# marvinx97/cloud

Measured on AMD Instinct MI355X. Metric: images/sec ResNet-50 via run() at 1/2/4/8 MI355X; run()→first-step latency, higher is better.
Workload: dtype bf16

## Files before the change

cloud_amd/config.py:

```python
from __future__ import annotations

import os
from dataclasses import dataclass


@dataclass(frozen=True)
class Var:
    name: str
    type: type
    default: object
    doc: str
    area: str


_VARS = [
    Var("CLOUD_AMD_JOBS_DIR", str, "./jobs", "where run() stages job directories", "launcher"),
    Var("CLOUD_AMD_HOME", str, "~/.cloud_amd", "per-user state: the job-id index (jobs/<id> -> job directory) that "
        "python -m cloud_amd.jobs uses to find a job from any directory", "launcher"),
    Var("CLOUD_AMD_STAGE_COPY", bool, False, "stage code files by copying too (default: code "
        "hard-linked, every other file copied; a running job then never sees in-place edits of its sources)", "launcher"),
    Var("CLOUD_AMD_CPU_AFFINITY", bool, True, "launcher pins each GPU rank to the cores of its GPU's NUMA node "
        "(KFD io_links + sysfs cpulist), split between the ranks on that node; 0 = leave placement to the OS",
        "launcher"),
    Var("CLOUD_AMD_NUMA_ROOT", str, "/sys/devices/system/node", "sysfs NUMA-node tree read for rank CPU placement "
# ... 27 lines not shown
        "core of ca_gemm256p8.h for large GEMMs), 'glds' (128 core only), 'vp8' (the two-phase 256 core whenever "
        "M, N >= 256), 'reg' (register staging); any other name selects 'auto'", "ops"),
    Var("CLOUD_AMD_WGRAD_BLOCKS", int, 512, "convolution weight gradients: split-K so that about this many "
        "workgroups run (tiles x splits); fewer splits = less fp32 slab traffic, more = fuller CUs", "ops"),
    Var("CLOUD_AMD_WGRAD_BLOCKS_SMALLM", int, 512, "convolution weight gradients with <= 128 output channels "
        "(ResNet stem, layers 1-2): split-K workgroup target", "ops"),
    Var("CLOUD_AMD_STEM_WGRAD_BLOCKS", int, 2048, "space-to-depth stem weight gradient (the last kernel of the "
        "backward pass): split-K workgroup target", "ops"),
    Var("CLOUD_AMD_DENSE_WGRAD_BLOCKS", int, 640, "dense-layer weight gradients (BERT): split-K workgroup target "
        "(round 4, same box: 640 -> 6,993 / 6,993 seq/s, 768 -> 6,962 / 6,952, 1024 -> 6,892 / 6,911, 512 -> "
        "6,865 / 6,896; profiles/r4_s36/)",
        "ops"),
    Var("CLOUD_AMD_DENSE_WGRAD_256", bool, False, "dense-layer weight gradients whose 256 x 256 tiles times a split "
        "count fill one round of the chip (BERT QKV / FFN) run on the two-phase 256 core with that split (measured "
        "3 % slower on BERT than the 128 core's 1024-workgroup split: 6,749 / 6,754 vs 6,952 / 6,940 seq/s)", "ops"),
    Var("CLOUD_AMD_TAPMASK", bool, True, "convolutions: tap-mask / incremental buffer-mode gather loaders; 0 keeps "
        "the general per-chunk decode loaders (A/B runs)", "ops"),
    Var("CLOUD_AMD_SPLIT_XCD", bool, True, "split-K GEMM/conv grids: give each XCD contiguous (split, tile) "
        "ranges so the tiles of one K chunk share an L2; 0 remaps tiles only (A/B runs)", "ops"),
    Var("CLOUD_AMD_BN_APPLY_BLOCKS", int, 0, "BatchNorm apply passes (fwd y/mask, bwd dz): total workgroups of "
        "the HBM stream; 0 = the reduction kernels' tiling", "ops"),
    Var("CLOUD_AMD_BN_APPLY_ILV", bool, True, "BatchNorm apply passes: 1 = RP-row groups dealt round-robin to "
        "the workgroups (one contiguous sweep); 0 = one contiguous row chunk per workgroup", "ops"),
    Var("CLOUD_AMD_CONV_TALL", bool, True, "<= 64-channel 3x3 convolutions (fwd, stride-1 dgrad): 256 x 64 tiles "
        "with 4 x 1 waves; 0 = 128 x 64 with 2 x 2 waves", "ops"),
    Var("CLOUD_AMD_STEM_LDS", bool, True, "space-to-depth stem convolution forward on the LDS-resident patch + filter "
        "kernel (csrc/include/ca_conv_stem.h); 0 = the implicit-GEMM row-segment loader", "ops"),
    Var("CLOUD_AMD_STEM_TALL", bool, True, "space-to-depth stem convolution on the tall 256 x 64 tiles too (0.88 -> "
        "0.72 ms per call at b1024); 0 = 128 x 64 tiles (A/B runs)", "ops"),
    Var("CLOUD_AMD_STEM_BWD_RECOMPUTE", bool, True, "ResNet stem tail backward: a statistics-only max-pool "
        "backward pass, then the BN-backward apply recomputes the pooled gradient per 2x2 block (the 112x112 "
        "gradient is never written: 3.3 GB fewer per step at b1024).  With the window loads issued ahead of "
        "any branch: 0.65 + 0.90 ms against 1.09 + 0.94 for write-then-apply, +0.8 % end to end "
        "(profiles/r4_s44/); 0 = write g and run the separate apply pass", "ops"),
    Var("CLOUD_AMD_BN_GROUPS_MAX", int, 512, "BatchNorm statistics: most groups of the first-level reduction of the "
        "per-tile partial rows (1..512; ~64 rows per group)", "ops"),
    Var("CLOUD_AMD_GEMM_LIB", str, "never", "plain bf16 GEMMs (bias / accumulate only, no fused epilogue): 'never' "
        "(default: every GEMM on the in-tree kernels, the same engine on every box and rank), 'auto' (diagnostic: "
        "times the in-tree kernel against hipBLASLt once per shape and keeps the faster), 'always' "
        "(ops/raw.py PlainGemmPolicy)", "ops"),
    Var("CLOUD_AMD_GEMM_PRW", bool, True, "forward 1x1 convolutions with N = 256, K = 64 (ResNet layer-1 conv3 "
        "and shortcut): persistent resident-weight core (csrc/include/ca_gemm_prw.h); 0 = the tiled 128 core",
        "ops"),
    Var("CLOUD_AMD_GEMM_PRWN", bool, True, "forward 1x1 convolutions N = 512 / K = 128 and N = 1024 / K = 256 with "
        "BN statistics (ResNet stage-2 / stage-3 conv3): the persistent core with the weight resident in column "
        "chunks (ca_gemm_prw.h); 0 = the tiled 128 core", "ops"),
    Var("CLOUD_AMD_SMALLK_SET", str, "", "bench/smallk_gemm.py shape set ('conv3': the conv3 expansions of "
        "stages 2-4)", "bench"),
    Var("CLOUD_AMD_EPI_PF", bool, True, "GEMM epilogues that read memory or run an activation (BN-statistics "
        "and inference-BN forward 1x1 convs, BERT bias/GELU/GELU'/beta dense layers): 4 staged output rows in flight per trip", "ops"),
    Var("CLOUD_AMD_EPI_PIPE", bool, True, "input-gradient GEMMs / convolutions with the BN-backward statistics "
        "epilogue: the next two output rows' operand loads are in flight under this pair's arithmetic and stores "
        "(ca_mfma_core.h gemm_epilogue); 0 = one pair at a time (A/B runs)", "ops"),
    Var("CLOUD_AMD_ATTN_FUSED_BWD", bool, True,"attention at S = 64 / 128: one workgroup per (batch, head) for "
        "the forward and a single fused backward kernel; 0 keeps the 64-query-block kernels", "ops"),
    Var("CLOUD_AMD_CONV_HALO_WGRAD", bool, True, "the weight gradient of the same 3x3 / 64-channel / width-56 "
        "convolutions on the LDS-resident kernel (ca_conv_halo.h conv3x3_halo_wgrad: 64 x 576 partial in registers, "
        "one fp32 slab per workgroup); 0 = implicit GEMM (A/B)", "ops"),
    Var("CLOUD_AMD_LN_BWD16", bool, False, "LayerNorm backward on 16-wave blocks, one row per wave, the block's "
        "partials summed by a fixed LDS tree (measured 2.8 % slower on BERT beside the weight-gradient side stream; "
        "default: 4-wave blocks walking four rows per wave)", "ops"),
    Var("CLOUD_AMD_GEMM_256X96", bool, True, "forward GEMMs whose 256 x 96 grid fills whole rounds while the 128 x "
        "128 grid leaves a partial one (BERT QKV, M = 8192, N = 2304) run on 256 x 96 tiles; 0 = off (A/B)", "ops"),
    Var("CLOUD_AMD_BN_FIN_RPG", int, 512, "BatchNorm statistics finalize: partial rows per group block (64-512)", "ops"),
    Var("CLOUD_AMD_BN_FIN_MERGED", bool, True, "BatchNorm statistics from many partial rows: group reduction and "
        "per-channel finalize in ONE launch (last block per 64 channels finalizes, agent-scope ticket); 0 = two "
        "launches (A/B runs)", "ops"),
    Var("CLOUD_AMD_CONV_HALO", int, 1, "3x3 / stride-1 / 64-channel convolutions at width 56 (ResNet-50 "
        "stage 1) forward and input gradient on the LDS-resident kernel (ca_conv_halo.h: input patch and all 9 taps "
        "in LDS, persistent grid); 0 = implicit-GEMM tiles, 2 = halo kernel without the software-pipelined "
        "fragment reads (A/B runs)", "ops"),
    Var("CLOUD_AMD_CONV_PATCH", bool, True, "3x3 / stride-1 / pad-1 convolutions with a 64-multiple gathered channel "
        "count, more than 64 output columns and W <= 28 (ResNet-50 stages 2-4), forward and input gradient, on the "
        "patch-fed core (ca_conv_patch.h: the tile's input rows go to LDS once per 64-channel chunk, not once per "
        "tap); 0 = tap-gathered implicit GEMM (A/B runs)", "ops"),
    Var("CLOUD_AMD_CONV_EPI_PF", bool, True, "implicit-GEMM forward convolutions with the BN-statistics epilogue, and "
        "with the inference BN + residual + ReLU epilogue: read 2 staged output rows from LDS before storing", "ops"),
    Var("CLOUD_AMD_INFER_FUSE", bool, True, "ResNet blocks and stem that are not training (eval mode, or a frozen "
        "Keras base) under torch.no_grad(): every BatchNorm (+ residual + ReLU) in the epilogue of its convolution "
        "(ops.conv_bn_act_infer, ca_conv_fwd_bn) and no BN-statistics partials; 0 = the per-layer route "
        "(convolution with statistics, then bn_apply)", "ops"),
    Var("CLOUD_AMD_SHAPE_LOG", str, None, "profiling: append one JSON line per GEMM/convolution launch (kind, M, N, "
        "K, minimum HBM bytes) to this file, for scripts/gemm_roofline.py", "ops"),
    Var("CLOUD_AMD_BN_FOLD", bool, True, "ResNet block backward: the bn3 / bn1 backward apply runs in the operand "
        "fetch of the 1x1 input-gradient GEMM that consumes it (ca_gemm_xa.h) instead of a separate pass", "ops"),
    Var("CLOUD_AMD_BN_FOLD_FWD", bool, True, "ResNet block forward: bn2's apply runs in conv3's operand fetch and "
        "bn3's (+ residual) in the next block's conv1 (ca_gemm_xa.h); the applied tensors are written once, by "
        "those GEMMs", "ops"),
    Var("CLOUD_AMD_BN_FOLD_MAX_N", int, 256, "BN fold sites kept: only GEMMs with K >= 2N and N <= this "
        "(ResNet-50 default: bn3 -> conv3 dgrad and bn3 -> next conv1 at stages 1-3, the stage-3 ones on the two-deep "
        "128 x 256 transform-A tiles, CLOUD_AMD_XA_N256=3: +0.6 / +1.0 % on two boxes, docs/performance.md round 6; "
        "4096 = every stage); the short-K sites (bn2 -> conv3, bn1 -> conv1 dgrad) measured slower than the separate "
        "pass, and stage 4 (N 512) +0.3 % below stages 1-3 only", "ops"),
    Var("CLOUD_AMD_BN_FOLD_WGRAD", bool, True, "bn3 -> conv3 fold at 64 input channels (ResNet stage 1): conv3's weight "
        "gradient runs in the same kernel as its input gradient (ca_gemm_xa.h mfma_gemm_xa_dw), so the BN-backward "
        "output dz3 is never written", "ops"),
    Var("CLOUD_AMD_BN_FOLD_DS", bool, False, "ResNet projection blocks, stages 2-4: the shortcut BN's backward apply "
        "runs in the operand fetch of the sparse strided shortcut input-gradient GEMM (ca_gemm_xa_bwd_strided); A/B",
        "ops"),
    Var("CLOUD_AMD_DS_SPARSE_DGRAD", bool, True, "ResNet projection blocks with a strided 1x1 shortcut: the "
        "shortcut's input gradient is written for its one non-empty output-parity class only, and conv1's input "
        "gradient accumulates into it reading the other pixels as zeros -- no zero-fill of 3/4 of dx and no read "
        "of those zeros", "ops"),
    Var("CLOUD_AMD_BN_FOLD_WGRAD_DS", bool, True, "stage-1 projection shortcut: its BN backward (gated by the block "
        "output's ReLU mask), the shortcut conv's input gradient and its weight gradient in one pass", "ops"),
    Var("CLOUD_AMD_BN_FOLD_WGRAD2", bool, False, "the same one-pass input + weight gradient for stage 2's conv3 "
# ... 166 lines not shown
```

csrc/bindings.cpp:

```cpp
#include <atomic>
#include <mutex>
#include <hip/hip_runtime.h>
#include <pybind11/pybind11.h>
#include <pybind11/stl.h>
#include <stdint.h>

#include <stdexcept>
#include <string>
#include <vector>

namespace py = pybind11;
typedef uint16_t bf16_t;

extern "C" {
int ca_sgd_step(float*, void*, int, float*, bf16_t*, const float*, const float*, long, int, int, hipStream_t);
int ca_adam_step(float*, void*, int, float*, float*, bf16_t*, const float*, const float*, long, int, int, hipStream_t);
int ca_rmsprop_step(float*, void*, int, float*, float*, bf16_t*, const float*, const float*, long, int, hipStream_t);
int ca_sumsq(const void*, int, long, float*, hipStream_t);
int ca_scale(void*, int, long, const float*, hipStream_t);
long ca_bn_workspace_floats(long, int);
int ca_bn_fwd(const bf16_t*, const bf16_t*, bf16_t*, long, int, const float*, const float*, float, float,
              float*, float*, float*, float*, float*, float*, int, uint8_t*, hipStream_t);
int ca_bn_apply(const bf16_t*, const bf16_t*, bf16_t*, long, int, const float*, int, hipStream_t);
int ca_bn_fwd_partials(const bf16_t*, const bf16_t*, bf16_t*, long, int, const float*, int, const float*, const float*,
// ... 21 lines not shown
                           hipStream_t);
int ca_gemm_xa_dw(const bf16_t*, const bf16_t*, const uint8_t*, const float*, const float*, const float*, long,
                  const bf16_t*, long, bf16_t*, long, int, int, int, float, const bf16_t*, const uint8_t*,
                  const bf16_t*, const uint8_t*, float*, const bf16_t*, float*, const bf16_t*, long, void*, int, float,
                  float*, int, hipStream_t);
int ca_dgrad_gemm(int, const bf16_t*, long, const bf16_t*, long, bf16_t*, long, int, int, int, float, const bf16_t*,
                  const uint8_t*, const bf16_t*, const uint8_t*, float*, hipStream_t, const bf16_t*, float*, int, int,
                  int);
int ca_conv_dgrad_bnstats(const bf16_t*, const bf16_t*, bf16_t*, int, int, int, int, int, int, int, int, int, int,
                          int, float, const bf16_t*, const uint8_t*, float*, hipStream_t);
int ca_u8_normalize(const uint8_t*, bf16_t*, long, int, const float*, const float*, hipStream_t);
int ca_stem_s2d(const bf16_t*, bf16_t*, int, int, int, int, int, int, int, hipStream_t);
int ca_softmax_xent(const void*, int, const int64_t*, int, int, float, float, float*, float*, void*, hipStream_t);
int ca_softmax_xent_batch(const void*, long, int, const int64_t*, int, int, float, float, float*, float*, void*, float*,
                          float,
                          hipStream_t);
int ca_maxpool_fwd(const bf16_t*, bf16_t*, uint8_t*, int, int, int, int, int, int, int, int, int, hipStream_t);
int ca_maxpool_bwd(const bf16_t*, const uint8_t*, bf16_t*, int, int, int, int, int, int, int, int, int, hipStream_t);
int ca_gap_fwd(const bf16_t*, void*, int, int, int, int, hipStream_t);
int ca_gap_bwd(const void*, int, bf16_t*, int, int, int, hipStream_t);
int ca_gmp_fwd(const bf16_t*, bf16_t*, float*, int, int, int, hipStream_t);
int ca_gmp_bwd(const void*, int, const bf16_t*, const bf16_t*, const float*, bf16_t*, int, int, int, hipStream_t);
int ca_gemm_bf16(int, const bf16_t*, long, const bf16_t*, long, bf16_t*, long, int, int, int, float*, float,
                 hipStream_t);
int ca_gemm_set_core(int);
int ca_gemm_set_xa_n256(int);
int ca_gemm_stat_rows(int, int, int, long, long, long);
int ca_bn_relu_maxpool_s2k3(const bf16_t*, const float*, bf16_t*, uint8_t*, int, int, int, int, int, int, hipStream_t);
int ca_maxpool_bnstats_parts(int, int, int, int);
int ca_maxpool_bwd_s2k3_bnstats(const bf16_t*, const bf16_t*, const uint8_t*, const bf16_t*, bf16_t*, float*, int, int,
                                int, int, int, int, hipStream_t);
int ca_maxpool_bwd_s2k3_bnapply(const bf16_t*, const bf16_t*, const uint8_t*, const bf16_t*, const float*, bf16_t*, int,
                                int, int, int, int, int, hipStream_t);
int ca_conv_fwd_ex(const bf16_t*, const bf16_t*, bf16_t*, int, int, int, int, int, int, int, int, int, int, int,
                   const float*, int, hipStream_t);
int ca_conv_fwd(const bf16_t*, const bf16_t*, bf16_t*, int, int, int, int, int, int, int, int, int, int, int, float*,
                hipStream_t);
int ca_conv_fwd_bn(const bf16_t*, const bf16_t*, bf16_t*, int, int, int, int, int, int, int, int, int, int, int,
                   const float*, const float*, const bf16_t*, int, hipStream_t);
int ca_conv_dgrad(const bf16_t*, const bf16_t*, bf16_t*, int, int, int, int, int, int, int, int, int, int, int, float,
                  hipStream_t, int);
int ca_conv_wgrad(const bf16_t*, const bf16_t*, void*, int, float, int, int, int, int, int, int, int, int, int, int,
                  int, int, float*, hipStream_t);
int ca_splitk_reduce(const float*, int, long, void*, int, float, hipStream_t);
int ca_grad_finalize_multi(const uint64_t*, const float*, int, hipStream_t);
int ca_cls_head_max_labels();
int ca_cls_head_fwd(const bf16_t*, long, const float*, const float*, float*, int, int, int, float, uint64_t,
                    hipStream_t);
int ca_cls_head_bwd(const float*, const bf16_t*, long, const float*, bf16_t*, float*, float*, int, int, int, float,
                    uint64_t, hipStream_t);
int ca_gemm_splitk(int, const bf16_t*, long, const bf16_t*, long, void*, int, float, int, int, int, int, float*,
                   hipStream_t);
int ca_gemm_splitk_effective(int, int);
int ca_gemm_ex(int, const bf16_t*, long, const bf16_t*, long, bf16_t*, long, int, int, int, float*, float, const float*,
               int, bf16_t*, const bf16_t*, long, hipStream_t);
long ca_ln_workspace_floats(long, int);
int ca_ln_fwd(const bf16_t*, const bf16_t*, const float*, const float*, bf16_t*, bf16_t*, float*, float*, long, int,
              float, float, uint64_t, float, uint64_t, const float*, hipStream_t);
int ca_ln_bwd(const bf16_t*, const bf16_t*, const float*, const float*, const float*, bf16_t*, bf16_t*, float*, float*,
              int, float*, long, int, float, uint64_t, float, uint64_t, hipStream_t, float*);
long ca_colsum_workspace_floats(long, int);
int ca_colsum(const bf16_t*, long, int, long, float*, int, float*, hipStream_t);
int ca_act_grad(const bf16_t*, long, int, const bf16_t*, bf16_t*, long, int, int, hipStream_t);
int ca_pad_cols(const void*, long, int, void*, int, long, long, int, hipStream_t);
int ca_slice_acc(const float*, long, void*, int, long, int, hipStream_t);
int ca_pad_cols_multi(const long*, int, hipStream_t);
int ca_splitk_bias_act(const float*, int, long, int, const float*, int, bf16_t*, hipStream_t);
int ca_embed_sum(const int32_t*, const int32_t*, const float*, const float*, const float*, bf16_t*, long, int, int, int,
                 hipStream_t);
int ca_embed_bwd(const bf16_t*, const int32_t*, const int32_t*, float*, float*, float*, long, int, int, int, int, int,
                 int, float*, unsigned*, hipStream_t);
int ca_dropout(const bf16_t*, bf16_t*, long, float, uint64_t, hipStream_t);
int ca_dropout_mask(uint8_t*, long, long, float, uint64_t, hipStream_t);
int ca_attn_fwd(const bf16_t*, bf16_t*, float*, const int*, int, int, int, float, float, uint64_t, int, hipStream_t);
int ca_attn_bwd(const bf16_t*, const bf16_t*, const bf16_t*, const float*, float*, bf16_t*, const int*, int, int, int,
                float, float, uint64_t, int, hipStream_t);
}

#define P(T, x) reinterpret_cast<T>(static_cast<uintptr_t>(x))
#define S(x) reinterpret_cast<hipStream_t>(static_cast<uintptr_t>(x))

static void check(int rc, const char* what) {
  if (rc != 0) {
    std::string msg = std::string(what) + " failed: ";
    if (rc > 0) msg += hipGetErrorString(static_cast<hipError_t>(rc));
    else if (rc == -3)
      msg += "an operand window of one GEMM block exceeds the 2 GiB reach of the buffer loads (split the batch or K)";
    else msg += "invalid arguments (code " + std::to_string(rc) + ")";
    throw std::runtime_error(msg);
  }
}

typedef unsigned long long u64;

static int stream_wait(u64 dst, u64 src) {
  static hipEvent_t ring[16];
  static std::atomic<int> next{0};
  static std::once_flag once;
  static hipError_t init_err = hipSuccess;
  std::call_once(once, [] {
    for (auto& e : ring) {
      const hipError_t rc = hipEventCreateWithFlags(&e, hipEventDisableTiming);
      if (rc != hipSuccess) init_err = rc;
    }
  });
  if (init_err != hipSuccess) return (int)init_err;
// ... 214 lines not shown
  });
  m.def("maxpool_bwd_s2k3_bnapply", [](u64 dy, u64 yp, u64 idx, u64 z, u64 coef, u64 dz, int N, int H, int W, int C,
                                       int OH, int OW, u64 s) {
    check(ca_maxpool_bwd_s2k3_bnapply(P(const bf16_t*, dy), P(const bf16_t*, yp), P(const uint8_t*, idx),
                                      P(const bf16_t*, z), P(const float*, coef), P(bf16_t*, dz), N, H, W, C, OH, OW,
                                      S(s)),
          "maxpool_bwd_s2k3_bnapply");
  });
  m.def("conv_fwd_ex", [](u64 x, u64 w, u64 y, int Nb, int H, int W, int Cin, int Cout, int KH, int KW, int sh,
                          int sw, int ph, int pw, u64 bias, int act, u64 s) {
    check(ca_conv_fwd_ex(P(const bf16_t*, x), P(const bf16_t*, w), P(bf16_t*, y), Nb, H, W, Cin, Cout, KH, KW, sh, sw,
                         ph, pw, P(const float*, bias), act, S(s)), "conv_fwd_ex");
  });
  m.def("conv_dgrad", [](u64 dy, u64 w, u64 dx, int Nb, int H, int W, int Cin, int Cout, int KH, int KW, int sh,
                         int sw, int ph, int pw, float beta, u64 s, int skip_empty) {
    check(ca_conv_dgrad(P(const bf16_t*, dy), P(const bf16_t*, w), P(bf16_t*, dx), Nb, H, W, Cin, Cout, KH, KW, sh, sw,
                        ph, pw, beta, S(s), skip_empty), "conv_dgrad");
  }, py::arg("dy"), py::arg("w"), py::arg("dx"), py::arg("Nb"), py::arg("H"), py::arg("W"), py::arg("Cin"),
        py::arg("Cout"), py::arg("KH"), py::arg("KW"), py::arg("sh"), py::arg("sw"), py::arg("ph"), py::arg("pw"),
        py::arg("beta"), py::arg("s"), py::arg("skip_empty") = 0);
  m.def("conv_wgrad", [](u64 dy, u64 x, u64 dw, int dw_bf16, float beta, int Nb, int H, int W, int Cin, int Cout,
                         int KH, int KW, int sh, int sw, int ph, int pw, int splits, u64 ws, u64 s) {
    check(ca_conv_wgrad(P(const bf16_t*, dy), P(const bf16_t*, x), P(void*, dw), dw_bf16, beta, Nb, H, W, Cin, Cout,
                        KH, KW, sh, sw, ph, pw, splits, P(float*, ws), S(s)), "conv_wgrad");
  });
  m.def("grad_finalize_multi", [](const std::vector<uint64_t>& jobs, const std::vector<float>& betas, u64 s) {
    const int n = (int)betas.size();
    if ((long)jobs.size() != 12L * n) throw std::runtime_error("grad_finalize_multi: 12 fields per job");
    check(ca_grad_finalize_multi(jobs.data(), betas.data(), n, S(s)), "grad_finalize_multi");
  });
  m.def("cls_head_max_labels", []() { return ca_cls_head_max_labels(); });
  m.def("cls_head_fwd", [](u64 pooled, long ldp, u64 wc, u64 bc, u64 logits, int B, int C, int L, float p, u64 seed,
                           u64 s) {
    check(ca_cls_head_fwd(P(const bf16_t*, pooled), ldp, P(const float*, wc), P(const float*, bc), P(float*, logits),
                          B, C, L, p, seed, S(s)), "cls_head_fwd");
  });
  m.def("cls_head_bwd", [](u64 dl, u64 pooled, long ldp, u64 wc, u64 dpre, u64 gwc, u64 gbc, int B, int C, int L,
                           float p, u64 seed, u64 s) {
    check(ca_cls_head_bwd(P(const float*, dl), P(const bf16_t*, pooled), ldp, P(const float*, wc), P(bf16_t*, dpre),
                          P(float*, gwc), P(float*, gbc), B, C, L, p, seed, S(s)), "cls_head_bwd");
  });
  m.def("splitk_reduce", [](u64 ws, int splits, long MN, u64 out, int out_bf16, float beta, u64 s) {
    check(ca_splitk_reduce(P(const float*, ws), splits, MN, P(void*, out), out_bf16, beta, S(s)), "splitk_reduce");
  });
  m.def("gemm_splitk", [](int layout, u64 A, long lda, u64 B, long ldb, u64 out, int out_bf16, float beta, int M,
                          int N, int K, int splits, u64 ws, u64 s) {
    check(ca_gemm_splitk(layout, P(const bf16_t*, A), lda, P(const bf16_t*, B), ldb, P(void*, out), out_bf16, beta,
                         M, N, K, splits, P(float*, ws), S(s)), "gemm_splitk");
  });
  m.def("gemm_stat_rows", [](int M, int N, int K, long lda, long ldb, long ldc) {
    return ca_gemm_stat_rows(M, N, K, lda, ldb, ldc);
  });
  m.def("gemm_splitk_effective", [](int K, int splits) { return ca_gemm_splitk_effective(K, splits); });
  m.def("gap_bwd", [](u64 dy, int dybf, u64 dx, int N, int HW, int C, u64 s) {
    check(ca_gap_bwd(P(const void*, dy), dybf, P(bf16_t*, dx), N, HW, C, S(s)), "gap_bwd");
  });
  m.def("gmp_fwd", [](u64 x, u64 y, u64 cnt, int N, int HW, int C, u64 s) {
    check(ca_gmp_fwd(P(const bf16_t*, x), P(bf16_t*, y), P(float*, cnt), N, HW, C, S(s)), "gmp_fwd");
  });
  m.def("gmp_bwd", [](u64 dy, int dy_bf16, u64 x, u64 y, u64 cnt, u64 dx, int N, int HW, int C, u64 s) {
    check(ca_gmp_bwd(P(const void*, dy), dy_bf16, P(const bf16_t*, x), P(const bf16_t*, y), P(const float*, cnt),
                     P(bf16_t*, dx), N, HW, C, S(s)), "gmp_bwd");
  });
  m.def("gemm_ex", [](int layout, u64 A, long lda, u64 B, long ldb, u64 C, long ldc, int M, int N, int K, u64 stats,
                      float beta, u64 bias, int act, u64 preact, u64 dact_src, long ld_aux, u64 s) {
    check(ca_gemm_ex(layout, P(const bf16_t*, A), lda, P(const bf16_t*, B), ldb, P(bf16_t*, C), ldc, M, N, K,
                     P(float*, stats), beta, P(const float*, bias), act, P(bf16_t*, preact), P(const bf16_t*, dact_src),
                     ld_aux, S(s)), "gemm_ex");
  });
  m.def("ln_workspace_floats", [](long M, int C) { return ca_ln_workspace_floats(M, C); });
  m.def("ln_fwd", [](u64 x, u64 res, u64 g, u64 b, u64 y, u64 h, u64 mu, u64 rs, long M, int C, float eps, float p_in,
                     u64 seed_in, float p_out, u64 seed_out, u64 s, u64 xb) {
    check(ca_ln_fwd(P(const bf16_t*, x), P(const bf16_t*, res), P(const float*, g), P(const float*, b), P(bf16_t*, y),
                    P(bf16_t*, h), P(float*, mu), P(float*, rs), M, C, eps, p_in, seed_in, p_out, seed_out,
                    P(const float*, xb), S(s)),
          "ln_fwd");
  });
  m.def("ln_bwd", [](u64 dy, u64 h, u64 mu, u64 rs, u64 g, u64 dh, u64 dx, u64 dg, u64 db, int acc, u64 ws, long M,
                     int C, float p_in, u64 seed_in, float p_out, u64 seed_out, u64 s, u64 dsum) {
    check(ca_ln_bwd(P(const bf16_t*, dy), P(const bf16_t*, h), P(const float*, mu), P(const float*, rs),
                    P(const float*, g), P(bf16_t*, dh), P(bf16_t*, dx), P(float*, dg), P(float*, db), acc,
                    P(float*, ws), M, C, p_in, seed_in, p_out, seed_out, S(s), P(float*, dsum)), "ln_bwd");
  }, py::arg("dy"), py::arg("h"), py::arg("mu"), py::arg("rs"), py::arg("g"), py::arg("dh"), py::arg("dx"),
        py::arg("dg"), py::arg("db"), py::arg("acc"), py::arg("ws"), py::arg("M"), py::arg("C"), py::arg("p_in"),
        py::arg("seed_in"), py::arg("p_out"), py::arg("seed_out"), py::arg("s"), py::arg("dsum") = 0);
  m.def("pad_cols", [](u64 in, long ld, int cols, u64 out, int cols_out, long rows, long rows_out, int eb, u64 s) {
    check(ca_pad_cols(P(const void*, in), ld, cols, P(void*, out), cols_out, rows, rows_out, eb, S(s)), "pad_cols");
  });
  m.def("splitk_bias_act", [](u64 ws, int splits, long M, int N, u64 bias, int act, u64 out, u64 s) {
    check(ca_splitk_bias_act(P(const float*, ws), splits, M, N, P(const float*, bias), act, P(bf16_t*, out), S(s)),
          "splitk_bias_act");
  });
  m.def("pad_cols_multi", [](std::vector<long> jobs, u64 s) {
    check(ca_pad_cols_multi(jobs.data(), (int)(jobs.size() / 8), S(s)), "pad_cols_multi");
  });
  m.def("slice_acc", [](u64 in, long ld_in, u64 out, int out_bf16, long rows, int cols, u64 s) {
    check(ca_slice_acc(P(const float*, in), ld_in, P(void*, out), out_bf16, rows, cols, S(s)), "slice_acc");
  });
  m.def("act_grad", [](u64 dy, long ld_dy, int N, u64 src, u64 out, long M, int Np, int act, u64 s) {
    check(ca_act_grad(P(const bf16_t*, dy), ld_dy, N, P(const bf16_t*, src), P(bf16_t*, out), M, Np, act, S(s)),
          "act_grad");
  });
  m.def("colsum_workspace_floats", [](long M, int N) { return ca_colsum_workspace_floats(M, N); });
  m.def("colsum", [](u64 x, long M, int N, long ld, u64 out, int acc, u64 ws, u64 s) {
    check(ca_colsum(P(const bf16_t*, x), M, N, ld, P(float*, out), acc, P(float*, ws), S(s)), "colsum");
  });
// ... 32 lines not shown
```

csrc/kernels/gemm.hip:

```cpp
#include <stdlib.h>
#include <string.h>

#include "ca_gemm256p8.h"
#include "ca_gemm_xa.h"

namespace {
using namespace ca;

template <int BM, int BN, template <int, int, int> class LA, template <int, int, int> class LB, int EPI, int NS>
__global__ void __launch_bounds__(256) dense_gemm_kernel(CoreParams P) {
  mfma_gemm_body<BM, BN, 2, 2, LA, LB, EPI, NS>(P);
}

template <int BM, int BN, template <int, int, int> class LA, template <int, int, int> class LB, int EPI>
__global__ void __launch_bounds__(256) __attribute__((amdgpu_waves_per_eu(4))) dense_gemm_glds_kernel(CoreParams P) {
  mfma_gemm_glds<BM, BN, 2, 2, LA, LB, EPI>(P);
}

template <int BM, int BN, template <int, int, int> class LA, template <int, int, int> class LB, int EPI>
__global__ void __launch_bounds__(256) __attribute__((amdgpu_waves_per_eu(4))) dense_gemm_glds_pf_kernel(CoreParams P) {
  mfma_gemm_glds<BM, BN, 2, 2, LA, LB, EPI, 4>(P);
}

bool epi_pf() {
  static const bool on = env_switch("CLOUD_AMD_EPI_PF", true);
  return on;
}

template <int EPI>
__global__ void __launch_bounds__(256) __attribute__((amdgpu_waves_per_eu(2))) dense_gemm_256x96_kernel(CoreParams P) {
  mfma_gemm_glds<256, 96, 2, 2, GDenseKC, GDenseKC, EPI>(P);
}

template <template <int, int, int> class LA, template <int, int, int> class LB, int EPI>
__global__ void __launch_bounds__(512) dense_gemm_256p8_kernel(CoreParams P) {
  mfma_gemm_256p8<LA, LB, EPI>(P);
}

int g_core_kind = -1;
int core_kind() {
  if (g_core_kind < 0) {
    const char* e = getenv("CLOUD_AMD_GEMM_CORE");
    g_core_kind = !e ? 5 : (e[0] == 'r' ? 0 : strcmp(e, "glds") == 0 ? 1 : strcmp(e, "vp8") == 0 ? 6 : 5);
  }
  return g_core_kind;
}
bool use_glds() { return core_kind() != 0; }

template <int BN, int KT, int NS, bool STATS>
__global__ void __launch_bounds__(512) prw_gemm_kernel(CoreParams P) {
  prw_gemm_body<BN, KT, NS, STATS>(P);
}

bool prw_enabled() {
  static const bool on = env_switch("CLOUD_AMD_GEMM_PRW", true);
  return on;
}

int cu_count() {
  static int n = -1;
  if (n < 0) {
    int dev = 0;
    hipDeviceProp_t prop;
    n = (hipGetDevice(&dev) == hipSuccess && hipGetDeviceProperties(&prop, dev) == hipSuccess &&
         prop.multiProcessorCount > 0)
            ? prop.multiProcessorCount
            : 256;
  }
  return n;
// ... 172 lines not shown
}

static bool use_256x96(const CoreParams& p, int splits) {
  static const bool en = env_switch("CLOUD_AMD_GEMM_256X96", true);
  if (!en || splits != 1 || p.N % 96 || p.M < 4096 || p.stats) return false;
  const long t96 = ((p.M + 255) / 256) * (p.N / 96), t128 = ((p.M + 127) / 128) * ((p.N + 127) / 128);
  return t96 >= 512 && tile_balance(t96) >= 0.999 && tile_balance(t128) < 0.95;
}

static bool use_256(const CoreParams& p, int splits) {
  if (core_kind() == 6) return p.M >= 256 && p.N >= 256;
  if (core_kind() != 5 || p.M < 256 || p.N < 256 || p.k_per_split < 512) return false;
  const long t = (long)((p.M + 255) / 256) * ((p.N + 255) / 256) * splits;
  if (splits > 1 && t >= 224 && t <= 256) return true;
  return t >= 256 && (tile_balance(t) >= 0.999 || (t >= 512 && tile_balance(t) >= 0.85));
}

template <int BM, int BN, template <int, int, int> class LA, template <int, int, int> class LB,
          template <int, int, int> class GA, template <int, int, int> class GB, int EPI>
int launch(const CoreParams& p0, int splits, hipStream_t s) {
  CoreParams p = p0;
  p.split_xcd = split_xcd_enabled();
  const int tiles = ((p.M + BM - 1) / BM) * ((p.N + BN - 1) / BN);
  const long span = (long)(p.k_per_split + BK > 256 ? p.k_per_split + BK : 256) * (p.lda > p.ldb ? p.lda : p.ldb) * 2;
  if (use_glds() && span >= (long)BUF_CAP) return -3;
  if constexpr (BM == 128 && BN == 128 && (EPI == EPI_BF16 || EPI == EPI_F32_PARTIAL || EPI == EPI_BF16_ST)) {
    if (use_256(p, splits)) {
      const int t256 = ((p.M + 255) / 256) * ((p.N + 255) / 256);
      constexpr bool AK = GA<BM, 1, 256>::KC, BKC = GB<BN, 1, 256>::KC;
      static_assert(AK || !BKC, "no layout pairs an M-contiguous A with a K-contiguous B");
      if constexpr (AK && BKC)
        dense_gemm_256p8_kernel<GDenseKC, GDenseKC, EPI><<<dim3(t256, 1, splits), 512, 0, s>>>(p);
      else if constexpr (AK && !BKC)
        dense_gemm_256p8_kernel<GDenseKC, GDenseNC, EPI><<<dim3(t256, 1, splits), 512, 0, s>>>(p);
      else if constexpr (!AK && !BKC)
        dense_gemm_256p8_kernel<GDenseNC, GDenseNC, EPI><<<dim3(t256, 1, splits), 512, 0, s>>>(p);
      CA_LAUNCH_CHECK();
      return 0;
    }
    if constexpr (EPI == EPI_BF16 && GA<BM, 1, 256>::KC && GB<BN, 1, 256>::KC) {
      if (use_glds() && use_256x96(p, splits)) {
        const int t = ((p.M + 255) / 256) * (p.N / 96);
        dense_gemm_256x96_kernel<EPI><<<dim3(t, 1, 1), 256, 0, s>>>(p);
        CA_LAUNCH_CHECK();
        return 0;
      }
    }
  }
  constexpr bool PLAIN = EPI == EPI_BF16;
  if constexpr (PLAIN || ((EPI == EPI_BF16_ST || EPI == EPI_BF16_AFF) && GA<BM, 1, 256>::KC && GB<BN, 1, 256>::KC)) {
    const bool want = !PLAIN || p.dact_src || p.act || p.beta != 0.f;
    if (want && use_glds() && epi_pf()) {
      dense_gemm_glds_pf_kernel<BM, BN, GA, GB, EPI><<<dim3(tiles, 1, splits), 256, 0, s>>>(p);
      CA_LAUNCH_CHECK();
      return 0;
    }
  }
  if (use_glds()) {
    dense_gemm_glds_kernel<BM, BN, GA, GB, EPI><<<dim3(tiles, 1, splits), 256, 0, s>>>(p);
    CA_LAUNCH_CHECK();
    return 0;
  }
  if (p.k_per_split <= BK)
    dense_gemm_kernel<BM, BN, LA, LB, EPI, 1><<<dim3(tiles, 1, splits), 256, 0, s>>>(p);
  else
    dense_gemm_kernel<BM, BN, LA, LB, EPI, 2><<<dim3(tiles, 1, splits), 256, 0, s>>>(p);
  CA_LAUNCH_CHECK();
  return 0;
}

static bool want_small_n(const CoreParams& p, int splits) {
  const long tm = (p.M + 127) / 128;
  const long t128 = tm * ((p.N + 127) / 128) * splits, t64 = tm * ((p.N + 63) / 64) * splits;
  return p.N <= 64 || (tile_balance(t128) < 0.8 && tile_balance(t64) > tile_balance(t128) + 0.1);
}

template <int BM, int BN, bool BKC, int EPI, int XM>
__global__ void __launch_bounds__(256) xa_gemm_kernel(CoreParams P, XaParams X) {
  mfma_gemm_xa<BM, BN, BKC, EPI, XM>(P, X);
}

template <int BM, int BN, bool BKC, int EPI, int XM>
__global__ void __launch_bounds__(512) __attribute__((amdgpu_waves_per_eu(4))) xa_gemm8_kernel(CoreParams P,
                                                                                              XaParams X) {
  mfma_gemm_xa<BM, BN, BKC, EPI, XM, 512>(P, X);
}

template <int BN, bool BKC, int EPI, int XM>
__global__ void __launch_bounds__(1024) __attribute__((amdgpu_waves_per_eu(4))) xa_gemm16d_kernel(CoreParams P,
                                                                                                 XaParams X) {
  mfma_gemm_xa_deep<BN, BKC, EPI, XM>(P, X);
}

template <int BM, int BN, bool BKC, int EPI, int XM>
__global__ void __launch_bounds__(1024) __attribute__((amdgpu_waves_per_eu(4))) xa_gemm16_kernel(CoreParams P,
                                                                                                XaParams X) {
  mfma_gemm_xa<BM, BN, BKC, EPI, XM, 1024>(P, X);
}

static bool xa_waves8_n64() {
  static const bool on = env_switch("CLOUD_AMD_XA_WAVES_N64", true);
  return on;
}
int g_xa_n256 = -1;
static int xa_n256() {
  if (g_xa_n256 < 0) {
// ... 348 lines not shown
    return -1;
  if ((bnz && !stats) || (bnz2 && (!bnz || !stats2 || !res_src))) return -1;
  CoreParams p = base_params(src0, lda, B, ldb, C, ldc, M, N, K);
  p.beta = beta;
  p.res_src = res_src;
  p.res_mask = res_mask;
  p.bnz = bnz;
  p.bnmask = bnmask;
  p.stats = stats;
  p.bnz2 = bnz2;
  p.stats2 = stats2;
  XaParams x{src0, src1, mask_in, c0, c1, c2, nullptr, nullptr, nullptr};
  const int tiles = (M + 127) / 128;
  const int depth = (N == 64 && K == 256) ? xa_dw_depth() : 0;
  static int w8 = -1;
  if (w8 < 0) {
    const char* e = getenv("CLOUD_AMD_XA_DW_WAVES");
    w8 = (e && e[0] == '8') ? 1 : 0;
  }
  bool deep = depth > 0 && !w8 && beta == 0.f && !res_src && !bnz2 && (bnz != nullptr) == (stats != nullptr);
  {
    const int b = (depth >= 2 && blocks > cu_count()) ? cu_count() : blocks;
    const long rows = (long)((tiles + b - 1) / b) * 128;
    long ld = lda > ldy ? lda : ldy;
    if (ldc > ld) ld = ldc;
    if (rows * ld * 2 >= (long)BUF_CAP) deep = false;
  }
  if (deep && depth >= 2 && blocks > cu_count()) blocks = cu_count();
  const int tpb = (tiles + blocks - 1) / blocks;
  const int g = (tiles + tpb - 1) / tpb;
  int rc;
  if (N == 64 && K == 64) rc = xa_dw_launch<1, 1>(p, x, Y, ldy, ws, g, tpb, s);
  else if (N == 64 && K == 128) rc = xa_dw_launch<2, 1>(p, x, Y, ldy, ws, g, tpb, s);
  else if (N == 64 && K == 256) {
    if (deep && depth == 1) rc = xa_dw_deep_launch<1>(p, x, Y, ldy, ws, g, tpb, s);
    else if (deep && depth == 2) rc = xa_dw_deep_launch<2>(p, x, Y, ldy, ws, g, tpb, s);
    else if (deep) rc = xa_dw_deep_launch<4>(p, x, Y, ldy, ws, g, tpb, s);
    else rc = w8 ? xa_dw_launch<4, 1, 64, 512>(p, x, Y, ldy, ws, g, tpb, s) : xa_dw_launch<4, 1>(p, x, Y, ldy, ws, g, tpb, s);
  }
  else if (K == 64 && N == 256) rc = xa_dw_launch<1, 4>(p, x, Y, ldy, ws, g, tpb, s);
  else if (N == 128 && K == 512) rc = xa_dw_launch<8, 1, 128, 512>(p, x, Y, ldy, ws, g, tpb, s);
  else return -1;
  if (rc < 0) return rc;
  rc = ca_splitk_reduce(ws, g, (long)K * N, dw, dw_bf16, dw_beta, s);
  return rc < 0 ? rc : g;
}

int ca_gemm_splitk_effective(int K, int splits) {
  int kps = (K / splits + BK - 1) / BK * BK;
  if (kps < BK) kps = BK;
  return (K + kps - 1) / kps;
}

int ca_gemm_splitk(int layout, const bf16_t* A, long lda, const bf16_t* B, long ldb, void* out, int out_bf16,
                   float beta, int M, int N, int K, int splits, float* ws, hipStream_t s) {
  if (M <= 0 || N < 8 || N % 8 != 0 || (layout == 2 && M % 8 != 0)) return -1;
  if (layout != 2 && K % 8 != 0) return -1;
  int kps = (K / splits + BK - 1) / BK * BK;
  if (kps < BK) kps = BK;
  splits = (K + kps - 1) / kps;
  CoreParams p = base_params(A, lda, B, ldb, ws, N, M, N, K);
  p.k_per_split = kps;
  p.split_stride = (long)M * N;
  int rc = dispatch<EPI_F32_PARTIAL>(layout, p, splits, s);
  if (rc || out_bf16 < 0) return rc;
  return ca_splitk_reduce(ws, splits, (long)M * N, out, out_bf16, beta, s);
}

}
```

Measured before the change: 16620.

## Add 3-deep LDS-DMA ring pipeline for split-K weight-gradient GEMMs

Adds a new GEMM core for dense split-K weight gradients on 128x128 tiles. It splits each K tile into halves and keeps two half-tiles in flight through a 3-stage LDS ring using direct buffer/global-to-LDS loads. The aim is to hide global memory latency behind MFMA compute, where the single-stage loop leaves it exposed. The kernel caps VGPRs at 128 and uses more LDS, which may cost occupancy. It is selected only when there are at least 16 tiles and splits are deep enough, and an env switch turns it off.

Measured after the change: 16620 (median of 4 runs). No clear change (+0.0%).

```diff
diff --git a/cloud_amd/config.py b/cloud_amd/config.py
--- a/cloud_amd/config.py
+++ b/cloud_amd/config.py
@@ -103,6 +103,10 @@
     Var("CLOUD_AMD_EPI_PIPE", bool, True, "input-gradient GEMMs / convolutions with the BN-backward statistics "
         "epilogue: the next two output rows' operand loads are in flight under this pair's arithmetic and stores "
         "(ca_mfma_core.h gemm_epilogue); 0 = one pair at a time (A/B runs)", "ops"),
+    Var("CLOUD_AMD_WGRAD_RING", bool, True, "dense split-K weight gradients on 128 x 128 tiles with >= 16 output "
+        "tiles and splits of >= 192 reduction rows (ResNet-50 stages 3-4 1x1, BERT): the workgroup keeps two K "
+        "half-tiles in flight in a 3-deep LDS-DMA ring (csrc/include/ca_gemm_ring.h); 0 = the single-stage loop "
+        "(A/B runs; slabs are bit-identical)", "ops"),
     Var("CLOUD_AMD_ATTN_FUSED_BWD", bool, True,"attention at S = 64 / 128: one workgroup per (batch, head) for "
         "the forward and a single fused backward kernel; 0 keeps the 64-query-block kernels", "ops"),
     Var("CLOUD_AMD_CONV_HALO_WGRAD", bool, True, "the weight gradient of the same 3x3 / 64-channel / width-56 "
diff --git a/csrc/bindings.cpp b/csrc/bindings.cpp
--- a/csrc/bindings.cpp
+++ b/csrc/bindings.cpp
@@ -97,6 +97,7 @@
 int ca_gemm_splitk(int, const bf16_t*, long, const bf16_t*, long, void*, int, float, int, int, int, int, float*,
                    hipStream_t);
 int ca_gemm_splitk_effective(int, int);
+int ca_wgrad_ring_depth(int, long);
 int ca_gemm_ex(int, const bf16_t*, long, const bf16_t*, long, bf16_t*, long, int, int, int, float*, float, const float*,
                int, bf16_t*, const bf16_t*, long, hipStream_t);
 long ca_ln_workspace_floats(long, int);
@@ -417,6 +418,7 @@
     return ca_gemm_stat_rows(M, N, K, lda, ldb, ldc);
   });
   m.def("gemm_splitk_effective", [](int K, int splits) { return ca_gemm_splitk_effective(K, splits); });
+  m.def("wgrad_ring_depth", [](int k_per_split, long tiles) { return ca_wgrad_ring_depth(k_per_split, tiles); });
   m.def("gap_bwd", [](u64 dy, int dybf, u64 dx, int N, int HW, int C, u64 s) {
     check(ca_gap_bwd(P(const void*, dy), dybf, P(bf16_t*, dx), N, HW, C, S(s)), "gap_bwd");
   });
diff --git a/csrc/include/ca_gemm_ring.h b/csrc/include/ca_gemm_ring.h
--- /dev/null
+++ b/csrc/include/ca_gemm_ring.h
@@ -0,0 +1,146 @@
+#pragma once
+#include <type_traits>
+
+#include "ca_mfma_core.h"
+
+namespace ca {
+
+inline bool wgrad_ring_enabled() {
+  static const bool on = env_switch("CLOUD_AMD_WGRAD_RING", true);
+  return on;
+}
+
+constexpr int WGRAD_RING_NS = 3;
+
+inline int wgrad_ring_pick(int k_per_split, long tiles) {
+  return (wgrad_ring_enabled() && (k_per_split + 31) / 32 >= 2 * WGRAD_RING_NS && tiles >= 16) ? WGRAD_RING_NS : 0;
+}
+
+__device__ __forceinline__ uint32_t lds_addr(const short* p) {
+  return __builtin_amdgcn_readfirstlane((uint32_t)(uintptr_t)(__attribute__((address_space(3))) const short*)p);
+}
+#pragma clang diagnostic push
+#pragma clang diagnostic ignored "-Winline-asm"
+__device__ __forceinline__ void ring_dma_buf(u32x4 rsrc, uint32_t voff, uint32_t dst) {
+  asm volatile("s_mov_b32 m0, %0\n\ts_nop 0\n\tbuffer_load_dwordx4 %1, %2, 0 offen lds"
+               :
+               : "s"(dst), "v"(voff), "s"(rsrc)
+               : "memory", "m0");
+}
+__device__ __forceinline__ void ring_dma_ptr(const bf16_t* src, uint32_t dst) {
+  asm volatile("s_mov_b32 m0, %0\n\ts_nop 0\n\tglobal_load_lds_dwordx4 %1, off"
+               :
+               : "s"(dst), "v"(src)
+               : "memory", "m0");
+}
+#pragma clang diagnostic pop
+template <class L>
+__device__ __forceinline__ u32x4 ring_rsrc(const L& l) {
+  if constexpr (loader_buf<L>::value) {
+    const uint64_t a = reinterpret_cast<uint64_t>(l.sbase);
+    return u32x4{(uint32_t)a, (uint32_t)(a >> 32) & 0xffffu, l.nrec, 0x00020000u};
+  } else {
+    return u32x4{0u, 0u, 0u, 0x00020000u};
+  }
+}
+#define CA_RING_DMA(L, l, r, i, k0, dst)                        \
+  do {                                                          \
+    if constexpr (loader_buf<L>::value)                         \
+      ring_dma_buf((r), (l).off((i), (k0)), lds_addr(dst));     \
+    else                                                        \
+      ring_dma_ptr((l).src((i), (k0)), lds_addr(dst));          \
+  } while (0)
+
+template <int BM, int BN, int WM, int WN, template <int, int, int> class LAT, template <int, int, int> class LBT,
+          int EPI, int NS>
+__device__ __forceinline__ void mfma_gemm_glds_ring(const CoreParams& P) {
+  constexpr int NT = WM * WN * 64;
+  constexpr int FM = BM / WM / 16, FN = BN / WN / 16;
+  constexpr int HK = BK / 2;
+  constexpr int A_H = BM * HK, B_H = BN * HK, HSTAGE = A_H + B_H;
+  constexpr int SMEM = NS * HSTAGE;
+  constexpr int CPA = BM * BK / 8 / NT, CPB = BN * BK / 8 / NT;
+  constexpr int HA = CPA / 2, HB = CPB / 2;
+  constexpr int PH = HA + HB;
+  using LA = LAT<BM, CPA, NT>;
+  using LB = LBT<BN, CPB, NT>;
+  static_assert(!LA::KC && !LB::KC, "ring core: reduction-major (NC) operands only");
+  static_assert(EPI == EPI_F32_PARTIAL, "ring core: fp32 slab epilogue only (it never touches LDS)");
+  static_assert(NS >= 3 && (NS - 2) * PH <= 40, "ring depth");
+  static_assert((BM * BK) % (16 * NT) == 0 && (BN * BK) % (16 * NT) == 0, "a half must be whole chunks per thread");
+  __shared__ __attribute__((aligned(16))) short smem[SMEM];
+
+  const int tid = threadIdx.x, lane = tid & 63, wave = tid >> 6;
+  const int wm = wave / WN, wn = wave % WN;
+  const int tiles_n = (P.N + BN - 1) / BN;
+  const BlkPos bp = blk_pos(P);
+  const int tm = bp.tile / tiles_n, tn = bp.tile % tiles_n;
+  const int m0 = tm * BM, n0 = tn * BN;
+  const int kbeg = bp.split * P.k_per_split;
+  int kend = kbeg + P.k_per_split;
+  if (kend > P.K) kend = P.K;
+  const int nh = 2 * ((kend - kbeg + BK - 1) / BK);
+
+  LA la(P, true, m0, tid);
+  LB lb(P, false, n0, tid);
+  const u32x4 ra = ring_rsrc(la);
+  const u32x4 rb = ring_rsrc(lb);
+
+  f4v acc[FM][FN];
+#pragma unroll
+  for (int i = 0; i < FM; ++i)
+#pragma unroll
+    for (int j = 0; j < FN; ++j) acc[i][j] = f4v{0.f, 0.f, 0.f, 0.f};
+
+  auto issue = [&](auto hpar, int hh, int st) {
+    constexpr int H = decltype(hpar)::value;
+    const int k0 = hh < nh ? kbeg + (hh >> 1) * BK : P.K;
+    short* base = smem + st * HSTAGE;
+#pragma unroll
+    for (int i = 0; i < HA; ++i) CA_RING_DMA(LA, la, ra, H * HA + i, k0, base + (i * NT + wave * 64) * 8);
+#pragma unroll
+    for (int i = 0; i < HB; ++i) CA_RING_DMA(LB, lb, rb, H * HB + i, k0, base + A_H + (i * NT + wave * 64) * 8);
+    if constexpr (H == 1) {
+      if constexpr (loader_stateful<LA>::value) la.advance();
+      if constexpr (loader_stateful<LB>::value) lb.advance();
+    }
+  };
+  auto compute = [&](int st) {
+    const short* As = smem + st * HSTAGE;
+    const short* Bs = As + A_H;
+    bf16x8 af[FM], bfr[FN];
+#pragma unroll
+    for (int i = 0; i < FM; ++i) af[i] = read_frag_sw<BM, false>(As, wm * (BM / WM) + i * 16, 0, lane);
+#pragma unroll
+    for (int j = 0; j < FN; ++j) bfr[j] = read_frag_sw<BN, false>(Bs, wn * (BN / WN) + j * 16, 0, lane);
+    mfma_acc<FM, FN>(acc, af, bfr);
+  };
+  using H0 = std::integral_constant<int, 0>;
+  using H1 = std::integral_constant<int, 1>;
+
+#pragma unroll
+  for (int q = 0; q < NS - 1; ++q) {
+    if (q & 1) issue(H1{}, q, q);
+    else issue(H0{}, q, q);
+  }
+  int cur = 0, fill = NS - 1;
+  auto step = [&](auto hfill, int s) {
+    vm_wait<(NS - 2) * PH>();
+    lgkm_wait0();
+    bar256();
+    issue(hfill, s + NS - 1, fill);
+    compute(cur);
+    cur = cur + 1 == NS ? 0 : cur + 1;
+    fill = fill + 1 == NS ? 0 : fill + 1;
+  };
+  for (int s = 0; s < nh; s += 2) {
+    step(std::integral_constant<int, (NS - 1) & 1>{}, s);
+    step(std::integral_constant<int, NS & 1>{}, s + 1);
+  }
+  vm_wait<0>();
+  lgkm_wait0();
+  bar256();
+  gemm_epilogue<BM, BN, WM, WN, EPI, SMEM, 1, FM, FN>(P, acc, smem, m0, n0, tm, tid);
+}
+
+}
diff --git a/csrc/kernels/gemm.hip b/csrc/kernels/gemm.hip
--- a/csrc/kernels/gemm.hip
+++ b/csrc/kernels/gemm.hip
@@ -2,6 +2,7 @@
 #include <string.h>
 
 #include "ca_gemm256p8.h"
+#include "ca_gemm_ring.h"
 #include "ca_gemm_xa.h"
 
 namespace {
@@ -15,6 +16,11 @@
 template <int BM, int BN, template <int, int, int> class LA, template <int, int, int> class LB, int EPI>
 __global__ void __launch_bounds__(256) __attribute__((amdgpu_waves_per_eu(4))) dense_gemm_glds_kernel(CoreParams P) {
   mfma_gemm_glds<BM, BN, 2, 2, LA, LB, EPI>(P);
+}
+
+template <template <int, int, int> class LA, template <int, int, int> class LB, int NS>
+__global__ void __launch_bounds__(256) __attribute__((amdgpu_num_vgpr(128))) dense_gemm_ring_kernel(CoreParams P) {
+  mfma_gemm_glds_ring<128, 128, 2, 2, LA, LB, EPI_F32_PARTIAL, NS>(P);
 }
 
 template <int BM, int BN, template <int, int, int> class LA, template <int, int, int> class LB, int EPI>
@@ -293,6 +299,13 @@
     const bool want = !PLAIN || p.dact_src || p.act || p.beta != 0.f;
     if (want && use_glds() && epi_pf()) {
       dense_gemm_glds_pf_kernel<BM, BN, GA, GB, EPI><<<dim3(tiles, 1, splits), 256, 0, s>>>(p);
+      CA_LAUNCH_CHECK();
+      return 0;
+    }
+  }
+  if constexpr (BM == 128 && BN == 128 && EPI == EPI_F32_PARTIAL && !GA<BM, 1, 256>::KC && !GB<BN, 1, 256>::KC) {
+    if (use_glds() && wgrad_ring_pick(p.k_per_split, tiles)) {
+      dense_gemm_ring_kernel<GA, GB, WGRAD_RING_NS><<<dim3(tiles, 1, splits), 256, 0, s>>>(p);
       CA_LAUNCH_CHECK();
       return 0;
     }
@@ -747,6 +760,8 @@
   return (K + kps - 1) / kps;
 }
 
+int ca_wgrad_ring_depth(int k_per_split, long tiles) { return use_glds() ? wgrad_ring_pick(k_per_split, tiles) : 0; }
+
 int ca_gemm_splitk(int layout, const bf16_t* A, long lda, const bf16_t* B, long ldb, void* out, int out_bf16,
                    float beta, int M, int N, int K, int splits, float* ws, hipStream_t s) {
   if (M <= 0 || N < 8 || N % 8 != 0 || (layout == 2 && M % 8 != 0)) return -1;
```
